# erikszasz/GaussianSplattingRegistration

Measured on AMD Instinct MI355X. Metric: Gaussians/sec through HEM level + ICP iters/sec, 2x5M-splat pair, higher is better.
Workload: dtype f32 (HEM) / f64 (ICP)

## Files before the change

gaussiansplattingregistration_amd/csrc/hem.hip:

```cpp
#include "gsr_common.h"
#include "gsr_math.h"
#include "gsr_normals.h"
#include "gsr_test_hooks.h"
#include "hem_device.h"
#include "hem_select.h"

#include <float.h>
#include <math.h>
#include <stdarg.h>
#include <stdlib.h>
#include <string.h>

#include <chrono>
#include <vector>

#include <rocprim/rocprim.hpp>

namespace gsr {

std::string& last_error() {
    static thread_local std::string s;
    return s;
}
int32_t fail(int32_t code, const char* fmt, ...) {
// ... 1774 lines not shown
        const unsigned g = gid[i];
        if ((int64_t)g >= n_global || (i > 0 && gid[i - 1] >= g)) atomicAdd(bad, 1u);
    }
}
__global__ __launch_bounds__(256) void k_gid_drop(int64_t n, const unsigned* __restrict__ bits, const int* __restrict__ wpre, unsigned* __restrict__ gid) {
    for (int64_t i = (int64_t)blockIdx.x * blockDim.x + threadIdx.x; i < n; i += (int64_t)gridDim.x * blockDim.x) {
        const unsigned g = gid[i];
        gid[i] = g - ((unsigned)wpre[g >> 5] + (unsigned)__popc(bits[g >> 5] & ((1u << (g & 31)) - 1u)));
    }
}
__global__ __launch_bounds__(256) void k_compact_u32(int64_t n, const int* __restrict__ keep, const int* __restrict__ pos, const unsigned* __restrict__ src,
                                                     unsigned* __restrict__ dst) {
    for (int64_t i = (int64_t)blockIdx.x * blockDim.x + threadIdx.x; i < n; i += (int64_t)gridDim.x * blockDim.x)
        if (keep[i]) dst[pos[i]] = src[i];
}
__global__ __launch_bounds__(256) void k_not_flag(int64_t n, const int* __restrict__ in, int* __restrict__ out) {
    for (int64_t i = (int64_t)blockIdx.x * blockDim.x + threadIdx.x; i < n; i += (int64_t)gridDim.x * blockDim.x) out[i] = in[i] ? 0 : 1;
}
__global__ void k_last_total(const int* __restrict__ pos_last, const int* __restrict__ flag_last, long long* __restrict__ out) { *out = (long long)*pos_last + *flag_last; }
__global__ void k_flip3(unsigned* __restrict__ w) { if (threadIdx.x < 3) w[threadIdx.x] = ~w[threadIdx.x]; }

__global__ __launch_bounds__(256) void k_valid(int64_t n, const float* __restrict__ xyz, const float* __restrict__ cov6,
                                               int* __restrict__ keep, const long long* __restrict__ n_dev, int* __restrict__ dropped,
                                               int* __restrict__ holes ) {
    if (n_dev) n = *n_dev;
    for (int64_t i = (int64_t)blockIdx.x * blockDim.x + threadIdx.x; i < n; i += (int64_t)gridDim.x * blockDim.x) {
        const float x = xyz[3 * i], y = xyz[3 * i + 1], z = xyz[3 * i + 2];
        s6 c = {cov6[6 * i], cov6[6 * i + 1], cov6[6 * i + 2], cov6[6 * i + 3], cov6[6 * i + 4], cov6[6 * i + 5]};
        const float d = det6(c);
        const bool bad = (x != x) || (y != y) || (z != z) || (d != d) || (d <= 0.0f);
        keep[i] = bad ? 0 : 1;
        if (bad && dropped) {
            const int slot = atomicAdd(dropped, 1);
            if (holes && slot < ERASE_MAX) holes[slot] = (int)i;
        }
    }
}

struct EraseArgs {
    float* arr[6];
    int w[6];
    uint8_t* flags;
    float* halo;
    int W;
    int tile;
    int max_tiles;
    const int* holes;
    const int* dropped;
// ... 288 lines not shown
    bool mstep_small = true;
    bool use_ell = true;
    int shard_rank = 0, shard_world = 1;
    gsr_allreduce_dev_fn shard_allreduce = nullptr;
    gsr_allgather_dev_fn shard_allgather = nullptr;
    void* shard_user = nullptr;
    DevBuf shard_send, shard_recv;
    bool sparse_path = false;
    DevBuf hitem, hfirst, part_cnt, Ac, cellStartC, cellStartI;
    DevBuf pcnt, poff, pair_child, pair_wl, spair_child, spair_wl, cstart, sumLw, oflag, pflag_in, oflag_in, prank_in, orank_in;
    DevBuf keep, kpos, scratch, draws, counters, rocprim_tmp, rocprim_tmp2, sh_tail, holes, erase_halo;
    int64_t stats[8] = {0, 0, 0, 0, 0, 0, 0, 0};
    int64_t stats_ex[8] = {0, 0, 0, 0, 0, 0, 0, 0};
    float phase_ms[8] = {0, 0, 0, 0, 0, 0, 0, 0};
    hipEvent_t ev[8] = {nullptr, nullptr, nullptr, nullptr, nullptr, nullptr, nullptr, nullptr};
    hipEvent_t evk[4] = {nullptr, nullptr, nullptr, nullptr};
    hipEvent_t evm[6] = {nullptr, nullptr, nullptr, nullptr, nullptr, nullptr};
    float kernel_ms[8] = {0, 0, 0, 0, 0, 0, 0, 0};
    struct Prologue { bool valid = false; GridParams gp; int P = 0, n_irr = 0, cblock = 0; int64_t n = 0; float ms = 0.0f; } pro;
    hipEvent_t ev_pro[2] = {nullptr, nullptr};
    int cblock = 0;
    DevBuf lvl;
    bool async_ok = true;
    bool last_level = false;
    hipStream_t side = nullptr;
    hipEvent_t ev_side = nullptr, ev_side_fork = nullptr;
    int round_trips = 0;
    int was_async = 0;
    float cell_target = 16.0f;
    int max_cells = 1 << 24;
};

namespace {

void rng_polymul(const unsigned* a, const unsigned* b, unsigned* out) {
    unsigned prod[61];
    for (int d = 0; d < 61; ++d) prod[d] = 0;
    for (int i = 0; i < 31; ++i) for (int j = 0; j < 31; ++j) prod[i + j] += a[i] * b[j];
    for (int d = 60; d >= 31; --d) { const unsigned c = prod[d]; prod[d - 3] += c; prod[d - 31] += c; }
    for (int d = 0; d < 31; ++d) out[d] = prod[d];
}
const unsigned* rng_xpow_table() {
    struct Table {
        unsigned tab[48 * 31];
        Table() {
            for (int j = 0; j < 31; ++j) tab[j] = j == 1 ? 1u : 0u;
// ... 93 lines not shown
    const unsigned long long seq = ++c->rb_seq;
    hipLaunchKernelGGL(k_collect, dim3(1), dim3(8), 0, c->stream, q, c->host_rb, seq);
    GSR_HIP(hipGetLastError());
    GSR_TRY(wait_round_trip(c, seq));
    for (int i = 0; i < q.n; ++i) out[i] = __atomic_load_n(c->host_rb + i, __ATOMIC_RELAXED);
    return GSR_OK;
}
int32_t read_back_level(gsr_hem_ctx* c, const LevelCollect& q, unsigned long long* out) {
    const unsigned long long seq = ++c->rb_seq;
    hipLaunchKernelGGL(k_level_collect, dim3(1), dim3(64), 0, c->stream, q, c->host_rb, seq);
    GSR_HIP(hipGetLastError());
    GSR_TRY(wait_round_trip(c, seq));
    for (int i = 0; i < LC_WORDS; ++i) out[i] = __atomic_load_n(c->host_rb + 16 + i, __ATOMIC_RELAXED);
    return GSR_OK;
}

#ifndef GSR_SCAN_BIG_N
#define GSR_SCAN_BIG_N (1 << 20)
#endif
using scan_cfg_big = rocprim::scan_config<256, 64, rocprim::block_load_method::block_load_transpose, rocprim::block_store_method::block_store_transpose,
                                          rocprim::block_scan_algorithm::using_warp_scan>;
using scan_cfg64_big = rocprim::scan_config<256, 32, rocprim::block_load_method::block_load_transpose, rocprim::block_store_method::block_store_transpose,
                                            rocprim::block_scan_algorithm::using_warp_scan>;
template <typename T>
int32_t exclusive_scan(gsr_hem_ctx* c, const T* in, T* out, int64_t n, bool side = false) {
    size_t bytes = 0;
    const hipStream_t s = side ? c->aux : c->stream;
    DevBuf& tmp = side ? c->rocprim_tmp2 : c->rocprim_tmp;
    if (n >= GSR_SCAN_BIG_N) {
        GSR_HIP(rocprim::exclusive_scan<scan_cfg_big>(nullptr, bytes, in, out, (T)0, (size_t)n, rocprim::plus<T>(), s));
        GSR_TRY(tmp.reserve(bytes));
        GSR_HIP(rocprim::exclusive_scan<scan_cfg_big>(tmp.p, bytes, in, out, (T)0, (size_t)n, rocprim::plus<T>(), s));
        return GSR_OK;
    }
    GSR_HIP(rocprim::exclusive_scan(nullptr, bytes, in, out, (T)0, (size_t)n, rocprim::plus<T>(), s));
    GSR_TRY(tmp.reserve(bytes));
    GSR_HIP(rocprim::exclusive_scan(tmp.p, bytes, in, out, (T)0, (size_t)n, rocprim::plus<T>(), s));
    return GSR_OK;
}

#ifndef GSR_SORT_RADIX_BITS
#define GSR_SORT_RADIX_BITS 10
#endif
#ifndef GSR_SORT_MERGE_LIMIT
#define GSR_SORT_MERGE_LIMIT (256 * 1024)
#endif
#ifndef GSR_SORT_BS
#define GSR_SORT_BS 1024
#endif
#ifndef GSR_SORT_IPT
// ... 135 lines not shown
        if (e == hipSuccess) e = hipEventCreateWithFlags(&c->ev_mjoin, hipEventDisableTiming);
        for (int i = 0; i < 4 && e == hipSuccess; ++i) e = hipEventCreate(&c->evp[i]);
        for (int i = 0; i < 2 && e == hipSuccess; ++i) e = hipEventCreate(&c->ev_pro[i]);
        if (e != hipSuccess) { delete c; return fail(GSR_E_HIP, "second stream: %s", hipGetErrorString(e)); }
    }
    {
        hipError_t e = hipHostMalloc((void**)&c->host_rb, 512, hipHostMallocMapped | hipHostMallocCoherent);
        if (e != hipSuccess) { c->host_rb = nullptr; delete c; return fail(GSR_E_HIP, "hipHostMalloc: %s", hipGetErrorString(e)); }
        memset(c->host_rb, 0, 512);
    }
    if (const char* s = getenv("GSR_HEM_ELL")) c->use_ell = atoi(s) != 0;
    if (const char* s = getenv("GSR_HEM_SUMLW")) c->sum_bucket = strcmp(s, "sort") != 0;
    if (const char* s = getenv("GSR_HEM_SPLIT")) c->split_heavy = atoi(s) != 0;
    if (const char* s = getenv("GSR_HEM_MSTEP_SMALL")) c->mstep_small = atoi(s) != 0;
    if (const char* s = getenv("GSR_HEM_MSTEP_SPLIT")) c->mstep_split = atoi(s) != 0;
    if (const char* s = getenv("GSR_HEM_SH_DIRECT")) c->sh_policy = atoi(s) != 0 ? 1 : 0;
    if (const char* s = getenv("GSR_HEM_SH_DIRECT_PAIRS")) c->sh_direct_pairs = (float)atof(s);
    if (const char* s = getenv("GSR_HEM_ROWLIST")) c->use_rowlist = atoi(s) != 0;
    if (const char* s = getenv("GSR_HEM_ROWLIST_MAX_MB")) c->rowlist_max = (size_t)(atof(s) * 1048576.0);
    if (const char* s = getenv("GSR_HEM_TIMING")) { const int v = atoi(s); c->timing = v < 0 ? 0 : (v > 2 ? 2 : v); }
    if (const char* s = getenv("GSR_HEM_SELECT_NP")) { const int v = atoi(s); c->select_np = v < 1 ? 1 : (v > SEL_NP ? SEL_NP : v); }
    if (const char* s = getenv("GSR_HEM_RB_POLL")) c->rb_poll = atoi(s) != 0;
    if (const char* s = getenv("GSR_HEM_ASYNC")) c->async_ok = atoi(s) != 0;
    if (const char* s = getenv("GSR_HEM_PARTITION_STAGE")) { const int v = atoi(s); if (v == 8192 || v == 6144 || v == 4096) c->partition_stage = v; }
    if (const char* s = getenv("GSR_HEM_PARTITION")) { c->partition_fixed = strcmp(s, "exact") != 0; c->partition_staged = strcmp(s, "walk") != 0; }
    if (const char* s = getenv("GSR_HEM_PARTITION_FACTOR")) c->partition_factor = atof(s);
    if (const char* s = getenv("GSR_HEM_CELL_TARGET")) { float v = (float)atof(s); if (v > 0.25f && v < 4096.0f) c->cell_target = v; }
    (void)hipFuncSetAttribute((const void*)k_bucket_sum, hipFuncAttributeMaxDynamicSharedMemorySize, 12 << 13);
    (void)hipFuncSetAttribute((const void*)k_bucket_hist, hipFuncAttributeMaxDynamicSharedMemorySize, SUM_MAX_BUCKETS * 4);
    (void)hipFuncSetAttribute((const void*)k_bucket_scatter, hipFuncAttributeMaxDynamicSharedMemorySize, SUM_MAX_BUCKETS * 4);
    (void)hipFuncSetAttribute((const void*)k_partition<0>, hipFuncAttributeMaxDynamicSharedMemorySize, SUM_MAX_BUCKETS * 4);
    (void)hipFuncSetAttribute((const void*)k_partition<8192>, hipFuncAttributeMaxDynamicSharedMemorySize, 1536 * 8 + 8192 * 8);
    (void)hipFuncSetAttribute((const void*)k_partition<6144>, hipFuncAttributeMaxDynamicSharedMemorySize, 3584 * 8 + 6144 * 8);
    (void)hipFuncSetAttribute((const void*)k_partition<4096>, hipFuncAttributeMaxDynamicSharedMemorySize, 5632 * 8 + 4096 * 8);
    (void)hipFuncSetAttribute((const void*)k_part_max, hipFuncAttributeMaxDynamicSharedMemorySize, 4 << 13);
    (void)hipFuncSetAttribute((const void*)k_part_acc, hipFuncAttributeMaxDynamicSharedMemorySize, 12 << 13);
    (void)hipFuncSetAttribute((const void*)k_erase_shift, hipFuncAttributeMaxDynamicSharedMemorySize, 12288 * 4);
    *out = c;
    return GSR_OK;
}

int32_t gsr_hem_destroy(gsr_hem_ctx* c) {
    if (!c) return GSR_OK;
    (void)hipSetDevice(c->device);
    unborrow_level0(c);
    for (DevBuf& b : c->spare) b.release();
// ... 478 lines not shown
            }
            GSR_TRY(gsr_comm_allreduce(c->comm, c->gbits.p, words, GSR_DT_U32, GSR_OP_SUM, (void*)st));
            hipLaunchKernelGGL(k_bits_popc, dim3(stride_grid(words)), blk, 0, st, words, c->gbits.as<unsigned>(), c->wcnt.as<int>());
            GSR_TRY(exclusive_scan<int>(c, c->wcnt.as<int>(), c->wpre.as<int>(), words));
            if (dropped > 0) {
                GSR_TRY(c->grank.reserve((size_t)n_pre * 4));
                hipLaunchKernelGGL(k_compact_u32, dim3(stride_grid(n_pre)), blk, 0, st, n_pre, c->keep.as<int>(), c->kpos.as<int>(), c->gid_next.as<unsigned>(), c->grank.as<unsigned>());
                c->gid_next.swap(c->grank);
            }
            if (O.n > 0) hipLaunchKernelGGL(k_gid_drop, dim3(stride_grid(O.n)), blk, 0, st, O.n, c->gbits.as<unsigned>(), c->wpre.as<int>(), c->gid_next.as<unsigned>());
            n_glob_next = n_pre_glob - dg;
        }
        c->part_stats[6] = dg;
        return GSR_OK;
    }
};

}

namespace {

constexpr int32_t GSR_RETRY_SYNC = -1000;

struct LevelRun {
    gsr_hem_ctx* c;
    hipStream_t st;
    Level& L;
    Level& O;
    const bool dbg_sync, part, sharded;
    bool spec = false;
    const int sh_policy;
    const int64_t n_own;
    int64_t n;
    const int F, RSH;
    PartLevel pl;
    const dim3 blk{256};
    dim3 grd;
    GridParams gp;
    int P_all = 0, P = 0, n_irr = 0;
    int* cnt = nullptr;
    long long* lvl = nullptr;
    const float4* rec_src = nullptr;
    bool ranks_forked = false, sh_pending = false, sh_launched = false, flags_forked = false;
    SelectArgs sa;
    size_t Pm = 1;
    int own_lo = 0, own_hi = 0;
    int64_t M = 0;
    unsigned long long cand = 0, cap_pairs = 0;
    const int64_t* seg = nullptr;
    const unsigned* pc = nullptr;
    const float* pw = nullptr;
    int bshift = 0, nbuckets = 0;
    int* overflow_flag = nullptr;
    bool fixed_tried = false;
    int64_t n_orph = 0, n_pre = 0, out_cap = 0;
    bool out_active = false;
    uint64_t rng_pos0 = 0;
    int64_t dropped = 0, P_glob = 0, O_glob = 0, n_pre_glob = 0, n_glob_next = 0;
    float pro_ms = 0.0f;

    LevelRun(gsr_hem_ctx* ctx, bool allow_async)
        : c(ctx), st(ctx->stream), L(ctx->cur), O(ctx->nxt), dbg_sync(getenv("GSR_HEM_DEBUG_SYNC") != nullptr), part(ctx->comm != nullptr),
          sharded(ctx->shard_world > 1 && ctx->shard_allreduce != nullptr), sh_policy(ctx->comm == nullptr ? ctx->sh_policy : 0), n_own(ctx->cur.n), n(ctx->cur.n), F(ctx->cur.F), RSH((ctx->cur.F + 3) & ~3) {
        spec = allow_async;
        pl.c = c; pl.st = st; pl.n_own = n_own;
        memset(&sa, 0, sizeof(sa));
    }
    ~LevelRun() {
        if (out_active) for (int i = 0; i < 5; ++i) { DevBuf* b = level_big(c->nxt, i); b->p = nullptr; b->cap = 0; b->swap(c->spare_out[i]); }
    }

    int32_t run(int64_t* n_out, int64_t* n_dropped);
    int32_t grid_phase();
    int32_t select_phase();
    int32_t sums_phase();
    int32_t sums_fixed();
    int32_t sums_exact();
    int32_t compact_pairs();
    int32_t output_ranks();
    int32_t open_output();
    int32_t mstep_phase();
    int32_t flags_and_validity();
    int32_t compact_erased(int64_t n_keep);
    int32_t erase_in_place(int64_t rows_bound, bool may_allocate, int64_t alloc_rows = 0);
    bool erase_on_device = false;
    int32_t launch_gather_sh(bool fork);
    int32_t widen_scan(const unsigned* cnt_in, int64_t* off, int64_t count);
    int32_t total_of(const int64_t* off, const unsigned* cnt_in, int64_t count, int64_t* out);
};

struct WidenU32 { __device__ __host__ int64_t operator()(unsigned v) const { return (int64_t)v; } };
int32_t LevelRun::widen_scan(const unsigned* cnt_in, int64_t* off, int64_t count) {
    auto in = rocprim::make_transform_iterator(cnt_in, WidenU32());
    size_t bytes = 0;
    if (count >= GSR_SCAN_BIG_N) {
        GSR_HIP(rocprim::exclusive_scan<scan_cfg64_big>(nullptr, bytes, in, off, (int64_t)0, (size_t)count, rocprim::plus<int64_t>(), st));
        GSR_TRY(c->rocprim_tmp.reserve(bytes));
        GSR_HIP(rocprim::exclusive_scan<scan_cfg64_big>(c->rocprim_tmp.p, bytes, in, off, (int64_t)0, (size_t)count, rocprim::plus<int64_t>(), st));
        return GSR_OK;
    }
    GSR_HIP(rocprim::exclusive_scan(nullptr, bytes, in, off, (int64_t)0, (size_t)count, rocprim::plus<int64_t>(), st));
    GSR_TRY(c->rocprim_tmp.reserve(bytes));
    GSR_HIP(rocprim::exclusive_scan(c->rocprim_tmp.p, bytes, in, off, (int64_t)0, (size_t)count, rocprim::plus<int64_t>(), st));
    return GSR_OK;
}
int32_t LevelRun::total_of(const int64_t* off, const unsigned* cnt_in, int64_t count, int64_t* out) {
    Collect q;
    q.n = 2;
    q.src[0] = off + (count - 1); q.bytes[0] = 8;
    q.src[1] = cnt_in + (count - 1); q.bytes[1] = 4;
    unsigned long long w[8];
    GSR_TRY(read_back(c, q, w));
    *out = (int64_t)w[0] + (int64_t)(unsigned)w[1];
    return GSR_OK;
}
// ... 41 lines not shown
            hipLaunchKernelGGL(k_flip3, dim3(1), dim3(64), 0, st, c->bbox.as<unsigned>());
            GSR_TRY(gsr_comm_allreduce(c->comm, c->bbox.p, 6, GSR_DT_U32, GSR_OP_MAX, (void*)st));
            hipLaunchKernelGGL(k_flip3, dim3(1), dim3(64), 0, st, c->bbox.as<unsigned>());
        }
        hipLaunchKernelGGL(k_hist, dim3(stride_grid(n) > 512 ? 512 : stride_grid(n)), blk, 0, st, n, L.xyz.as<float>(), c->bbox.as<unsigned>(), c->hist.as<unsigned>(),
                           (const long long*)nullptr);
        if (part) GSR_TRY(gsr_comm_allreduce(c->comm, c->hist.p, 3 * HIST_BINS, GSR_DT_U32, GSR_OP_SUM, (void*)st));
        hipLaunchKernelGGL(k_grid_params, dim3(1), dim3(64), 0, st, c->bbox.as<unsigned>(), c->hist.as<unsigned>(), part ? c->n_global : n, c->cell_target,
                           c->max_cells, c->gparams.as<GridParams>(), (const long long*)nullptr);
        static_assert(sizeof(GridParams) == 40, "GridParams is read back as five 8-byte words");
        Collect q;
        q.n = 7;
        for (int i = 0; i < 5; ++i) { q.src[i] = (const char*)c->gparams.p + 8 * i; q.bytes[i] = 8; }
        q.src[5] = c->bbox.as<unsigned>() + 6; q.src[6] = c->bbox.as<unsigned>() + 7;
        q.bytes[5] = q.bytes[6] = 4;
        unsigned long long w[8];
        GSR_TRY(read_back(c, q, w));
        memcpy(&gp, w, sizeof(gp));
        P_all = (int)(unsigned)w[5]; n_irr = (int)(unsigned)w[6];
    }
    overflow_flag = cnt + 12;
    c->stats[5] = gp.ncells;
    GSR_TRY(c->pflag_in.reserve(n * 4)); GSR_TRY(c->oflag_in.reserve(n * 4)); GSR_TRY(c->prank_in.reserve(n * 4)); GSR_TRY(c->orank_in.reserve(n * 4));
    if (!part && c->aux && c->ev_pre) {
        GSR_HIP(hipEventRecord(c->ev_fork, st)); GSR_HIP(hipStreamWaitEvent(c->aux, c->ev_fork, 0));
        hipLaunchKernelGGL(k_flags_in, grd, blk, 0, c->aux, n, n_own, L.is_parent.as<uint8_t>(), c->pflag_in.as<int>(), c->oflag_in.as<int>());
        GSR_TRY(exclusive_scan<int>(c, c->pflag_in.as<int>(), c->prank_in.as<int>(), n, true));
        GSR_HIP(hipEventRecord(c->ev_pre, c->aux));
        ranks_forked = true;
    }

    rec_src = c->rec.as<float4>();
    if (part) {
        GSR_TRY(pl.halo(gp, L, F, n));
        grd = dim3(stride_grid(n));
        rec_src = c->rec_loc.as<float4>();
    }
    GSR_TRY(c->keys.reserve(n * 4)); GSR_TRY(c->idx.reserve(n * 4)); GSR_TRY(c->skeys.reserve(n * 4)); GSR_TRY(c->order.reserve(n * 4));
    if (part) {
        GSR_TRY(c->perm.reserve(n * 4));
        hipLaunchKernelGGL(k_iota, grd, blk, 0, st, n, c->idx.as<unsigned>());
        GSR_TRY(sort_pairs<unsigned>(c, c->gid_loc.as<unsigned>(), c->skeys.as<unsigned>(), c->idx.as<unsigned>(), c->perm.as<unsigned>(), n, bits_for(c->n_global + 1)));
        hipLaunchKernelGGL(k_keys_rec, grd, blk, 0, st, n, rec_src, c->perm.as<unsigned>(), c->gparams.as<GridParams>(), c->keys.as<unsigned>(), c->idx.as<unsigned>());
    } else
        hipLaunchKernelGGL(k_keys, grd, blk, 0, st, n, L.xyz.as<float>(), c->gparams.as<GridParams>(), c->keys.as<unsigned>(), c->idx.as<unsigned>());
    GSR_TRY(sort_pairs<unsigned>(c, c->keys.as<unsigned>(), c->skeys.as<unsigned>(), c->idx.as<unsigned>(), c->order.as<unsigned>(), n,
                                 bits_for(gp.ncells)));
// ... 144 lines not shown
        if (sparse) {
            if (!spec) {
                const size_t Cm = (size_t)(cand > 0 ? cand : 1);
                GSR_TRY(c->sp_child.reserve(Cm * 4)); GSR_TRY(c->sp_wl.reserve(Cm * 4));
                cap_pairs = (unsigned long long)(std::min(c->sp_child.cap, c->sp_wl.cap) / 4);
            }
            sa.cap_pairs = cap_pairs;
            sa.poff = c->coff.as<int64_t>(); sa.pair_child = c->sp_child.as<unsigned>(); sa.pair_wl = c->sp_wl.as<float>();
            GSR_TIME1(c->evk[2], st);
            GSR_CHECKPOINT("spans + ordering");
            GSR_LAUNCH_SELECT(SEL_SPARSE);
            GSR_CHECKPOINT("k_select<SPARSE>");
            GSR_TIME1(c->evk[3], st);
        } else {
            GSR_TIME1(c->evk[0], st);
            GSR_LAUNCH_SELECT(SEL_COUNT);
            GSR_TIME1(c->evk[1], st);
        }
        GSR_TRY(widen_scan(c->pcnt.as<unsigned>(), c->poff.as<int64_t>(), P));
        if (!spec) GSR_TRY(total_of(c->poff.as<int64_t>(), c->pcnt.as<unsigned>(), P, &M));
        if ((spec || M > 0) && sparse && sa.heavy_blocks)
            hipLaunchKernelGGL(k_join_parts, dim3(1024), blk, 0, st, sa.nheavy, sa.porder, c->coff.as<int64_t>(), sa.hfirst, sa.part_cnt,
                               c->pcap.as<unsigned>(), sa.part_p, c->sp_child.as<unsigned>(), c->sp_wl.as<float>());
        if (!sh_launched) { GSR_TRY(launch_gather_sh(c->aux2 != nullptr)); sh_launched = true; }
        if (spec || M > 0) {
            if (!sparse) {
                const size_t Mm = (size_t)(M > 0 ? M : 1);
                GSR_TRY(c->pair_child.reserve(Mm * 4)); GSR_TRY(c->pair_wl.reserve(Mm * 4));
                sa.poff = c->poff.as<int64_t>(); sa.pair_child = c->pair_child.as<unsigned>(); sa.pair_wl = c->pair_wl.as<float>();
                if (sa.heavy_blocks)
                    hipLaunchKernelGGL(k_fill_const<int>, dim3(1), dim3(1), 0, st, (int64_t)1, sa.hq + 1, (int)(SEL_HEAVY_BLOCKS * WPB));
                GSR_TIME1(c->evk[2], st);
                GSR_LAUNCH_SELECT(SEL_FILL);
                GSR_TIME1(c->evk[3], st);
            }
        }
        c->sparse_path = sparse;
        c->stats_ex[1] = sparse ? 1 : 0;
    } else if (spec) {
        return GSR_RETRY_SYNC;
    }
#undef GSR_LAUNCH_SELECT
    c->stats[1] = M;
    GSR_CHECKPOINT("selection");
    GSR_TIME(c->ev[2], st);
    return GSR_OK;
}
// ... 158 lines not shown
        if (need > 0) {
            for (int i = 0; i < 5; ++i) {
                DevBuf* b = level_big(O, i);
                b->swap(c->spare_out[i]);
                b->p = c->out_ptr[i] ? c->out_ptr[i] : c->out_ptr[0]; b->cap = (size_t)-1;
            }
            out_active = true;
        }
    }
    GSR_TRY(O.reserve(need, F));
    out_cap = out_active ? std::min<int64_t>(c->out_rows, n + (int64_t)P) : need;
    if (spec) out_cap = std::min(out_cap, need);
    O.n = spec ? 0 : n_pre; O.F = F;
    if (spec)
        hipLaunchKernelGGL(k_level_tail, dim3(1), dim3(1), 0, st, n, P, c->orank_in.as<int>(), c->oflag_in.as<int>(), (long long)out_cap, lvl, cnt + 2);
    return GSR_OK;
}

int32_t LevelRun::mstep_phase() {
    const long long* n_pre_dev = spec ? lvl : nullptr;
    const int* sh_mode = reinterpret_cast<const int*>(lvl + 3);
    rng_pos0 = c->rng_pos;
    const int64_t n_draw = spec ? out_cap : n_pre;
    if (!part && c->aux && n_draw > 0) {
        GSR_HIP(hipEventRecord(c->ev_fork, st)); GSR_HIP(hipStreamWaitEvent(c->aux, c->ev_fork, 0));
        GSR_TRY(O.is_parent.reserve((size_t)n_draw));
        GSR_TRY(draw_flags_raw(c, n_draw, O.is_parent.as<uint8_t>(), c->aux, n_pre_dev));
        GSR_HIP(hipEventRecord(c->ev_join, c->aux));
        flags_forked = true;
    }
    if (!sh_launched) { GSR_TRY(launch_gather_sh(false)); sh_launched = true; }
    if (sh_pending) { GSR_HIP(hipStreamWaitEvent(st, c->ev_sh_join, 0)); sh_pending = false; }
    if (P > 0) {
        MstepArgs ma;
        memset(&ma, 0, sizeof(ma));
        ma.geo = c->geo.as<float4>(); ma.RSH = RSH;
        ma.sh_mode_p = sh_mode; ma.sh_own = L.sh.as<float>(); ma.sh_sorted = c->shs.as<float>();
        ma.sh_last = part ? 0xffffffffu : (unsigned)(n - 1); ma.sh_tail = c->sh_tail.as<float>();
        ma.pair_child = pc; ma.pair_wl = pw;
        ma.P = P; ma.F = F;
        ma.small = c->mstep_small ? 1 : 0;
        const unsigned* mporder = (spec || M > 0) ? c->porder.as<unsigned>() : nullptr;
        ma.xcd = mporder ? 1 : 0;
        ma.nheavy = mporder ? cnt + 8 : nullptr;
        GSR_TRY(c->mhdr.reserve(Pm * sizeof(MstepHeader)));
        const bool msplit = spec || M > MSTEP_SEG;
        if (msplit) {
// ... 3 lines not shown
            GSR_TRY(c->mh_scratch.reserve(cap_items * (size_t)(16 + RSH) * 4));
        }
        unsigned* hcount = (unsigned*)cnt;
        hipLaunchKernelGGL(k_mstep_headers, dim3(stride_grid(P)), blk, 0, st, P, mporder, c->plist.as<unsigned>(), seg,
                           c->pcnt.as<unsigned>(), c->order.as<unsigned>(), c->prank_in.as<int>(), c->A.as<float4>(), own_lo, own_hi,
                           c->mhdr.as<MstepHeader>(), (unsigned*)cnt + 15, (unsigned)MSTEP_SEG, msplit ? hcount : (unsigned*)nullptr,
                           c->mh_list.as<uint4>(), c->mh_items.as<uint2>());
        ma.hdr = c->mhdr.as<MstepHeader>();
        ma.split = c->mstep_split ? 1 : 0;
        ma.hcount = hcount; ma.hlist = c->mh_list.as<uint4>(); ma.hitems = c->mh_items.as<uint2>(); ma.hscratch = c->mh_scratch.as<float>();
        ma.o_xyz = O.xyz.as<float>(); ma.o_color = O.color.as<float>(); ma.o_cov6 = O.cov6.as<float>();
        ma.o_opacity = O.opacity.as<float>(); ma.o_weight = O.weight.as<float>(); ma.o_sh = O.sh.as<float>();
        const int nq = RSH >> 2;
        hipStream_t hst = st;
        if (msplit && c->aux) {
            GSR_HIP(hipEventRecord(c->ev_mfork, st)); GSR_HIP(hipStreamWaitEvent(c->aux, c->ev_mfork, 0));
            hst = c->aux;
        }
#define GSR_LAUNCH_MSTEP(G)                                                                                              \
    {                                                                                                                    \
        if (msplit && hst != st) {                                                                                       \
            hipLaunchKernelGGL((k_mstep<G, 1, true>), dim3(2048), dim3(64), 0, hst, ma);                                 \
            hipLaunchKernelGGL(k_mstep_heavy_finish, dim3(256), dim3(64), 0, hst, ma);                                   \
            GSR_HIP(hipEventRecord(c->ev_mjoin, hst));                                                                   \
        }                                                                                                                \
        hipLaunchKernelGGL((k_mstep<G, 1>), dim3(8 * ceil_div(ceil_div(P, MSTEP_K), 8)), dim3(64), 0, st, ma);           \
        if (msplit && hst == st) {                                                                                       \
            hipLaunchKernelGGL((k_mstep<G, 1, true>), dim3(2048), dim3(64), 0, st, ma);                                  \
            hipLaunchKernelGGL(k_mstep_heavy_finish, dim3(256), dim3(64), 0, st, ma);                                    \
        }                                                                                                                \
    }
        GSR_TIME1(c->evm[0], st);
        if (nq == 0) { GSR_LAUNCH_MSTEP(0) }
        else if (nq <= 1 * MSTEP_NV) { GSR_LAUNCH_MSTEP(1) }
        else if (nq <= 2 * MSTEP_NV) { GSR_LAUNCH_MSTEP(2) }
        else if (nq <= 4 * MSTEP_NV) { GSR_LAUNCH_MSTEP(4) }
        else if (nq <= 8 * MSTEP_NV) { GSR_LAUNCH_MSTEP(8) }
        else if (nq <= 16 * MSTEP_NV) { GSR_LAUNCH_MSTEP(16) }
        else { GSR_LAUNCH_MSTEP(32) }
#undef GSR_LAUNCH_MSTEP
        if (msplit && hst != st) GSR_HIP(hipStreamWaitEvent(st, c->ev_mjoin, 0));
        GSR_TIME1(c->evm[1], st);
    }
    hipLaunchKernelGGL(k_orphan_rows, dim3(stride_grid(n_own)), blk, 0, st, n_own, P, c->oflag_in.as<int>(), c->orank_in.as<int>(), L.xyz.as<float>(), L.color.as<float>(),
                       L.cov6.as<float>(), L.opacity.as<float>(), L.weight.as<float>(), L.sh.as<float>(), F, O.xyz.as<float>(), O.color.as<float>(),
                       O.cov6.as<float>(), O.opacity.as<float>(), O.weight.as<float>(), O.sh.as<float>(), (int64_t)(spec ? out_cap : n_pre));
// ... 8 lines not shown
                               c->order.as<unsigned>(), c->prank_in.as<int>(), c->shard_send.as<float>(), O.xyz.as<float>(), O.color.as<float>(),
                               O.cov6.as<float>(), O.opacity.as<float>(), O.weight.as<float>(), O.sh.as<float>());
        GSR_HIP(hipStreamSynchronize(st));
        if (c->shard_allgather(c->shard_send.p, c->shard_recv.p, (int64_t)chunk_bytes, c->shard_user) != 0)
            return fail(GSR_E_INVALID, "gsr_hem_run_level: all-gather callback failed (merged components)");
        for (int r = 0; r < W; ++r) {
            if (r == c->shard_rank) continue;
            const int lo = (int)((int64_t)P * r / W), hi = (int)((int64_t)P * (r + 1) / W);
            if (hi > lo)
                hipLaunchKernelGGL((k_shard_rows<false>), dim3(stride_grid((int64_t)(hi - lo) * RW)), blk, 0, st, lo, hi - lo, F, c->plist.as<unsigned>(),
                                   c->order.as<unsigned>(), c->prank_in.as<int>(), c->shard_recv.as<float>() + (size_t)r * chunk * RW, O.xyz.as<float>(),
                                   O.color.as<float>(), O.cov6.as<float>(), O.opacity.as<float>(), O.weight.as<float>(), O.sh.as<float>());
        }
    }
    P_glob = P; O_glob = n_orph;
    if (part) GSR_TRY(pl.global_ranks(P, n_pre, P_glob, O_glob));
    n_pre_glob = P_glob + O_glob;
    GSR_CHECKPOINT("M-step + orphans");
    GSR_TIME(c->ev[4], st);
    return GSR_OK;
}

int32_t LevelRun::erase_in_place(int64_t rows_bound, bool may_allocate, int64_t alloc_rows) {
    const int tile0 = std::min(256, 12288 / std::max(F, 6));
    const auto halo_bytes = [&](int64_t rows) { return (size_t)((rows + tile0 - 1) / tile0 + 1) * ERASE_MAX * ((size_t)(14 + F) * 4 + 1) + 64; };
    {
        const size_t need = halo_bytes(rows_bound);
        if (!may_allocate && c->erase_halo.cap < need) {
            hipLaunchKernelGGL(k_fill_const<long long>, dim3(1), dim3(1), 0, st, (int64_t)1, lvl + 4, (long long)0);
            return GSR_OK;
        }
    }
    erase_on_device = true;
    EraseArgs ea;
    memset(&ea, 0, sizeof(ea));
    float* arrs[6] = {O.xyz.as<float>(), O.color.as<float>(), O.cov6.as<float>(), O.opacity.as<float>(), O.weight.as<float>(), O.sh.as<float>()};
    const int ws[6] = {3, 3, 6, 1, 1, F};
    for (int q = 0; q < 6; ++q) { ea.arr[q] = arrs[q]; ea.w[q] = ws[q]; }
    ea.flags = O.is_parent.as<uint8_t>();
    ea.W = 14 + F;
    ea.tile = std::min(256, 12288 / std::max(F, 6));
    ea.max_tiles = (int)((rows_bound + ea.tile - 1) / ea.tile) + 1;
    GSR_TRY(c->erase_halo.reserve(halo_bytes(std::max(rows_bound, alloc_rows))));
    ea.halo = c->erase_halo.as<float>();
    ea.holes = c->holes.as<int>(); ea.dropped = cnt + 3; ea.n_pre_p = lvl; ea.n_keep_out = lvl + 4;
    const int g = std::min(ea.max_tiles, 2048);
    hipLaunchKernelGGL(k_erase_save, dim3(g), blk, 0, st, ea);
    hipLaunchKernelGGL(k_erase_shift, dim3(g), blk, (size_t)12288 * 4, st, ea);
    GSR_HIP(hipGetLastError());
    return GSR_OK;
}

int32_t LevelRun::compact_erased(int64_t n_keep) {
    Level& T = c->tmp;
    const dim3 g2(stride_grid(n_pre));
    GSR_TRY(T.reserve(n_keep, F));
    T.n = n_keep; T.F = F;
    const int* keep = c->keep.as<int>();
    const int* pos = c->kpos.as<int>();
    hipLaunchKernelGGL(k_compact_rows, dim3(stride_grid(n_pre * 3)), blk, 0, st, n_pre, 3, keep, pos, O.xyz.as<float>(), T.xyz.as<float>());
    hipLaunchKernelGGL(k_compact_rows, dim3(stride_grid(n_pre * 3)), blk, 0, st, n_pre, 3, keep, pos, O.color.as<float>(), T.color.as<float>());
    hipLaunchKernelGGL(k_compact_rows, dim3(stride_grid(n_pre * 6)), blk, 0, st, n_pre, 6, keep, pos, O.cov6.as<float>(), T.cov6.as<float>());
    hipLaunchKernelGGL(k_compact_rows, g2, blk, 0, st, n_pre, 1, keep, pos, O.opacity.as<float>(), T.opacity.as<float>());
    hipLaunchKernelGGL(k_compact_rows, g2, blk, 0, st, n_pre, 1, keep, pos, O.weight.as<float>(), T.weight.as<float>());
    if (F > 0)
        hipLaunchKernelGGL(k_compact_rows4, dim3(stride_grid(n_pre * ((F + 3) / 4))), blk, 0, st, n_pre, F, keep, pos, O.sh.as<float>(), T.sh.as<float>());
    hipLaunchKernelGGL(k_compact_bytes, g2, blk, 0, st, n_pre, keep, pos, O.is_parent.as<uint8_t>(), T.is_parent.as<uint8_t>());
    if (out_active) {
        const size_t row_bytes[5] = {12, 12, 24, 4, (size_t)F * 4};
        for (int i = 0; i < 5; ++i)
            if (row_bytes[i] > 0 && n_keep > 0)
                GSR_HIP(hipMemcpyAsync(level_big(O, i)->p, level_big(T, i)->p, (size_t)n_keep * row_bytes[i], hipMemcpyDeviceToDevice, st));
        O.weight.swap(T.weight); O.is_parent.swap(T.is_parent);
        O.n = n_keep;
    } else
        O.swap(T);
    return GSR_OK;
}

int32_t LevelRun::flags_and_validity() {
    if (part) {
        GSR_TRY(c->allflags.reserve((size_t)(n_pre_glob > 0 ? n_pre_glob : 1)));
        GSR_TRY(draw_flags_raw(c, n_pre_glob, c->allflags.as<uint8_t>()));
        if (n_pre > 0)
            hipLaunchKernelGGL(k_gather_bytes, dim3(stride_grid(n_pre)), blk, 0, st, n_pre, c->gid_next.as<unsigned>(), c->allflags.as<uint8_t>(), O.is_parent.as<uint8_t>());
    } else if (flags_forked) {
        GSR_HIP(hipStreamWaitEvent(st, c->ev_join, 0));
    } else {
        GSR_TRY(draw_flags(c, O));
    }
    dropped = 0;
    if (n_pre > 0) {
        GSR_TRY(c->keep.reserve(n_pre * 4)); GSR_TRY(c->kpos.reserve(n_pre * 4));
        const dim3 g2(stride_grid(n_pre));
        GSR_TRY(c->holes.reserve(ERASE_MAX * 4));
        hipLaunchKernelGGL(k_valid, g2, blk, 0, st, n_pre, O.xyz.as<float>(), O.cov6.as<float>(), c->keep.as<int>(), (const long long*)nullptr, cnt + 3, c->holes.as<int>());
        if (part) GSR_TRY(exclusive_scan<int>(c, c->keep.as<int>(), c->kpos.as<int>(), n_pre));
        {
            Collect q;
            q.n = 2;
            q.src[0] = cnt + 3; q.src[1] = cnt + 15;
            q.bytes[0] = q.bytes[1] = 4;
            unsigned long long w[8];
            GSR_TRY(read_back(c, q, w));
            dropped = (int64_t)(unsigned)w[0];
            if (P > 0) c->stats_ex[5] = (int64_t)(unsigned)w[1];
        }
        if (dropped > 0 && dropped <= ERASE_MAX && !part) {
            hipLaunchKernelGGL(k_fill_const<long long>, dim3(1), dim3(1), 0, st, (int64_t)1, lvl, (long long)n_pre);
            GSR_TRY(erase_in_place(n_pre, true, n));
            O.n = n_pre - dropped;
        } else if (dropped > 0) {
            if (!part) GSR_TRY(exclusive_scan<int>(c, c->keep.as<int>(), c->kpos.as<int>(), n_pre));
            GSR_TRY(compact_erased(n_pre - dropped));
        }
    }
    n_glob_next = n_pre_glob;
    if (part) GSR_TRY(pl.drop_erased(O, n_pre, n_pre_glob, dropped, n_glob_next));
    GSR_CHECKPOINT("flags + validity");
    return GSR_OK;
}

int32_t LevelRun::run(int64_t* n_out, int64_t* n_dropped) {
    memset(c->stats, 0, sizeof(c->stats));
    memset(c->stats_ex, 0, sizeof(c->stats_ex));
    memset(c->part_stats, 0, sizeof(c->part_stats));
    c->stats[6] = n;
    if (part) {
        pl.W = gsr_comm_world(c->comm); pl.me = gsr_comm_rank(c->comm);
        const unsigned code = c->shard_world > 1 ? 4u : (pl.W > 8 ? 3u : (n >= (1ll << 30) ? 2u : 0u));
        GSR_TRY(pl.agree_on_preconditions(n, code));
    }
    if (n >= (1ll << 30)) return fail(GSR_E_INVALID, "gsr_hem_run_level: %lld components (the candidate records carry the sorted position in 30 bits)", (long long)n);
    if (n == 0) {
        if (n_out) *n_out = 0;
        if (n_dropped) *n_dropped = 0;
        return GSR_OK;
    }
    spec = spec && !part && !sharded && !dbg_sync && c->sum_bucket && c->partition_fixed && !c->partition_overflowed && c->partition_factor == 0.0 &&
           c->split_heavy && getenv("GSR_HEM_SPARSE_GB") == nullptr && c->aux != nullptr &&
           std::min(c->sp_child.cap, c->sp_wl.cap) >= (size_t)4096 && std::min(c->spair_child.cap / sizeof(slot_t), c->spair_wl.cap / 4) >= (size_t)4096;
    grd = dim3(stride_grid(n));
    GSR_TIME1(c->ev[0], st);
    GSR_TRY(grid_phase());
    GSR_TRY(select_phase());
    GSR_TRY(sums_phase());
    GSR_TRY(output_ranks());
    GSR_TRY(open_output());
    GSR_TRY(mstep_phase());

    unsigned long long w[LC_WORDS];
    bool have_next = false;
    const bool want_pro = !c->last_level;
    const int cb_next = c->cblock ^ 1;
    LevelCollect q;
    memset(&q, 0, sizeof(q));
    q.cnt = cnt; q.gp = c->gparams.as<GridParams>(); q.bbox = c->bbox.as<unsigned>();
    if (P > 0) { q.coff = c->coff.as<int64_t>(); q.pcap = c->pcap.as<unsigned>(); q.poff = c->poff.as<int64_t>(); q.pcnt = c->pcnt.as<unsigned>(); q.P = P; }
    if (spec) {
        if (flags_forked) GSR_HIP(hipStreamWaitEvent(st, c->ev_join, 0));
        GSR_TRY(c->keep.reserve((size_t)out_cap * 4)); GSR_TRY(c->kpos.reserve((size_t)out_cap * 4));
        GSR_TRY(c->holes.reserve(ERASE_MAX * 4));
        hipLaunchKernelGGL(k_valid, dim3(stride_grid(out_cap)), blk, 0, st, out_cap, O.xyz.as<float>(), O.cov6.as<float>(), c->keep.as<int>(), (const long long*)lvl, cnt + 3,
                           c->holes.as<int>());
        GSR_TRY(erase_in_place(out_cap, false));
        GSR_TIME1(c->ev[5], st);
        if (want_pro) GSR_TRY(enqueue_prologue(c, O, out_cap, erase_on_device ? lvl + 4 : lvl, cb_next));
        q.lvl = lvl;
        GSR_TRY(read_back_level(c, q, w));
        if (w[LC_FLAGS] != 0ull) return GSR_RETRY_SYNC;
        cand = w[LC_CAND]; M = (int64_t)w[LC_PAIRS]; n_orph = (int64_t)w[LC_ORPHANS]; n_pre = (int64_t)w[LC_NPRE];
        c->stats[4] = (int64_t)cand; c->stats[1] = M; c->stats[2] = n_orph;
        c->stats_ex[3] = (int64_t)w[LC_HEAVY]; c->stats_ex[4] = (int64_t)w[LC_ITEMS]; c->stats_ex[5] = (int64_t)w[LC_MAXPAIRS];
        c->rng_pos = rng_pos0 + (uint64_t)n_pre;
        O.n = n_pre;
        P_glob = P; O_glob = n_orph; n_pre_glob = n_pre; n_glob_next = n_pre;
        dropped = (int64_t)w[LC_DROPPED];
        have_next = dropped == 0 || (erase_on_device && dropped <= ERASE_MAX);
        if (have_next) O.n = n_pre - dropped;
        else if (dropped <= ERASE_MAX) {
            GSR_TRY(erase_in_place(n_pre, true, out_cap));
            O.n = n_pre - dropped;
        } else {
            GSR_TRY(exclusive_scan<int>(c, c->keep.as<int>(), c->kpos.as<int>(), n_pre));
            GSR_TRY(compact_erased(n_pre - dropped));
        }
    } else {
        GSR_TRY(flags_and_validity());
// ... 251 lines not shown
```

Baseline: 578.6 million.

## Add single-block scan for small inputs and fold side-stream forks on small levels

Adds a one-block, 1024-thread warp-scan kernel that replaces the rocprim exclusive scans (including the widening u32→i64 scan) when the input fits in 64K items and is 16-byte aligned. This avoids rocprim's temp-size query and multi-kernel launches. Levels under 128K components skip the aux-stream fork for the flags scan and the gather-SH launch. The parent-flag draw is moved onto the heavy-mstep side stream so one fork/join serves both. The erase kernel launch is skipped when the halo buffer is too small, with k_valid clearing the keep count itself. The aim is to cut launch, event and stream-sync overhead on the many small coarse levels, at the cost of more code paths and some lost overlap.

```diff
diff --git a/gaussiansplattingregistration_amd/csrc/hem.hip b/gaussiansplattingregistration_amd/csrc/hem.hip
--- a/gaussiansplattingregistration_amd/csrc/hem.hip
+++ b/gaussiansplattingregistration_amd/csrc/hem.hip
@@ -1820,8 +1820,10 @@
 
 __global__ __launch_bounds__(256) void k_valid(int64_t n, const float* __restrict__ xyz, const float* __restrict__ cov6,
                                                int* __restrict__ keep, const long long* __restrict__ n_dev, int* __restrict__ dropped,
-                                               int* __restrict__ holes ) {
+                                               int* __restrict__ holes ,
+                                               long long* __restrict__ clear_p ) {
     if (n_dev) n = *n_dev;
+    if (clear_p && blockIdx.x == 0 && threadIdx.x == 0) *clear_p = 0;
     for (int64_t i = (int64_t)blockIdx.x * blockDim.x + threadIdx.x; i < n; i += (int64_t)gridDim.x * blockDim.x) {
         const float x = xyz[3 * i], y = xyz[3 * i + 1], z = xyz[3 * i + 2];
         s6 c = {cov6[6 * i], cov6[6 * i + 1], cov6[6 * i + 2], cov6[6 * i + 3], cov6[6 * i + 4], cov6[6 * i + 5]};
@@ -2156,6 +2158,7 @@
     int cblock = 0;
     DevBuf lvl;
     bool async_ok = true;
+    bool fold = true;
     bool last_level = false;
     hipStream_t side = nullptr;
     hipEvent_t ev_side = nullptr, ev_side_fork = nullptr;
@@ -2295,10 +2298,85 @@
                                           rocprim::block_scan_algorithm::using_warp_scan>;
 using scan_cfg64_big = rocprim::scan_config<256, 32, rocprim::block_load_method::block_load_transpose, rocprim::block_store_method::block_store_transpose,
                                             rocprim::block_scan_algorithm::using_warp_scan>;
+#ifndef GSR_SCAN_ONE_N
+#define GSR_SCAN_ONE_N 65536
+#endif
+constexpr int SCAN_ONE_TILES = GSR_SCAN_ONE_N / (16 * 256);
+static_assert(SCAN_ONE_TILES >= 1 && SCAN_ONE_TILES <= 16 && SCAN_ONE_TILES * 16 * 256 == GSR_SCAN_ONE_N, "GSR_SCAN_ONE_N: 16 waves x whole tiles of 256 items, at most 16 each");
+template <typename TIn, typename TOut, int TILES>
+__global__ __launch_bounds__(1024) void k_scan_one(int n, const TIn* __restrict__ in, TOut* __restrict__ out) {
+    static_assert(sizeof(TIn) == 4 && (sizeof(TOut) == 4 || sizeof(TOut) == 8), "k_scan_one: 4-byte items, 4- or 8-byte sums");
+    using WaveScan = rocprim::warp_scan<TOut, 64>;
+    __shared__ typename WaveScan::storage_type s_scan[16];
+    __shared__ TOut s_tot[16];
+    const int lane = threadIdx.x & 63, wv = threadIdx.x >> 6;
+    const int per_wave = (n + 16 * 256 - 1) / (16 * 256) * 256;
+    const int base = wv * per_wave + lane * 4;
+    uint4 v[TILES];
+#pragma unroll
+    for (int t = 0; t < TILES; ++t) {
+        const int i = base + t * 256;
+        const bool mine = t * 256 < per_wave;
+        if (mine && i + 3 < n) {
+            v[t] = *reinterpret_cast<const uint4*>(in + i);
+        } else {
+            v[t].x = mine && i < n ? (unsigned)in[i] : 0u;
+            v[t].y = mine && i + 1 < n ? (unsigned)in[i + 1] : 0u;
+            v[t].z = mine && i + 2 < n ? (unsigned)in[i + 2] : 0u;
+            v[t].w = mine && i + 3 < n ? (unsigned)in[i + 3] : 0u;
+        }
+    }
+    TOut mine_sum = 0;
+#pragma unroll
+    for (int t = 0; t < TILES; ++t) mine_sum = mine_sum + ((TOut)(TIn)v[t].x + (TOut)(TIn)v[t].y + (TOut)(TIn)v[t].z + (TOut)(TIn)v[t].w);
+    {
+        TOut inc, tot;
+        WaveScan().inclusive_scan(mine_sum, inc, tot, s_scan[wv]);
+        if (lane == 0) s_tot[wv] = tot;
+    }
+    __syncthreads();
+#pragma unroll
+    for (int t = 0; t < TILES; ++t) asm volatile("" : "+v"(v[t].x), "+v"(v[t].y), "+v"(v[t].z), "+v"(v[t].w));
+    TOut carry = 0;
+    for (int u = 0; u < wv; ++u) carry = carry + s_tot[u];
+#pragma unroll
+    for (int t = 0; t < TILES; ++t) {
+        const int i = base + t * 256;
+        if (!(t * 256 < per_wave)) break;
+        const TOut s = (TOut)(TIn)v[t].x + (TOut)(TIn)v[t].y + (TOut)(TIn)v[t].z + (TOut)(TIn)v[t].w;
+        TOut inc, tot;
+        WaveScan().inclusive_scan(lane == 0 ? s + carry : s, inc, tot, s_scan[wv]);
+        carry = tot;
+        if (i >= n) continue;
+        TOut e[4];
+        e[0] = inc - s;
+        e[1] = e[0] + (TOut)(TIn)v[t].x; e[2] = e[1] + (TOut)(TIn)v[t].y; e[3] = e[2] + (TOut)(TIn)v[t].z;
+        if (i + 3 < n) {
+            if constexpr (sizeof(TOut) == 4) {
+                *reinterpret_cast<uint4*>(out + i) = make_uint4((unsigned)e[0], (unsigned)e[1], (unsigned)e[2], (unsigned)e[3]);
+            } else {
+                *reinterpret_cast<ulonglong2*>(out + i) = make_ulonglong2((unsigned long long)e[0], (unsigned long long)e[1]);
+                *reinterpret_cast<ulonglong2*>(out + i + 2) = make_ulonglong2((unsigned long long)e[2], (unsigned long long)e[3]);
+            }
+        } else {
+#pragma unroll
+            for (int k = 0; k < 4; ++k) if (i + k < n) out[i + k] = e[k];
+        }
+    }
+}
+template <typename TIn, typename TOut>
+bool scan_one(gsr_hem_ctx* c, const TIn* in, TOut* out, int64_t n, hipStream_t s) {
+    constexpr int TILES = sizeof(TOut) == 4 ? SCAN_ONE_TILES : (SCAN_ONE_TILES + 1) / 2;
+    if (!c->fold || n <= 0 || n > (int64_t)TILES * 16 * 256 || (((uintptr_t)in | (uintptr_t)out) & 15u) != 0 || (const void*)in == (const void*)out) return false;
+    hipLaunchKernelGGL((k_scan_one<TIn, TOut, TILES>), dim3(1), dim3(1024), 0, s, (int)n, in, out);
+    return true;
+}
+
 template <typename T>
 int32_t exclusive_scan(gsr_hem_ctx* c, const T* in, T* out, int64_t n, bool side = false) {
     size_t bytes = 0;
     const hipStream_t s = side ? c->aux : c->stream;
+    if (scan_one<T, T>(c, in, out, n, s)) return GSR_OK;
     DevBuf& tmp = side ? c->rocprim_tmp2 : c->rocprim_tmp;
     if (n >= GSR_SCAN_BIG_N) {
         GSR_HIP(rocprim::exclusive_scan<scan_cfg_big>(nullptr, bytes, in, out, (T)0, (size_t)n, rocprim::plus<T>(), s));
@@ -2480,6 +2558,7 @@
     if (const char* s = getenv("GSR_HEM_SELECT_NP")) { const int v = atoi(s); c->select_np = v < 1 ? 1 : (v > SEL_NP ? SEL_NP : v); }
     if (const char* s = getenv("GSR_HEM_RB_POLL")) c->rb_poll = atoi(s) != 0;
     if (const char* s = getenv("GSR_HEM_ASYNC")) c->async_ok = atoi(s) != 0;
+    if (const char* s = getenv("GSR_HEM_FOLD")) c->fold = atoi(s) != 0;
     if (const char* s = getenv("GSR_HEM_PARTITION_STAGE")) { const int v = atoi(s); if (v == 8192 || v == 6144 || v == 4096) c->partition_stage = v; }
     if (const char* s = getenv("GSR_HEM_PARTITION")) { c->partition_fixed = strcmp(s, "exact") != 0; c->partition_staged = strcmp(s, "walk") != 0; }
     if (const char* s = getenv("GSR_HEM_PARTITION_FACTOR")) c->partition_factor = atof(s);
@@ -3004,6 +3083,9 @@
 
 constexpr int32_t GSR_RETRY_SYNC = -1000;
 
+#ifndef GSR_INLINE_N
+#define GSR_INLINE_N (128 * 1024)
+#endif
 struct LevelRun {
     gsr_hem_ctx* c;
     hipStream_t st;
@@ -3024,6 +3106,8 @@
     long long* lvl = nullptr;
     const float4* rec_src = nullptr;
     bool ranks_forked = false, sh_pending = false, sh_launched = false, flags_forked = false;
+    bool flags_joined = false;
+    bool small_level = false;
     SelectArgs sa;
     size_t Pm = 1;
     int own_lo = 0, own_hi = 0;
@@ -3065,6 +3149,10 @@
     int32_t flags_and_validity();
     int32_t compact_erased(int64_t n_keep);
     int32_t erase_in_place(int64_t rows_bound, bool may_allocate, int64_t alloc_rows = 0);
+    size_t erase_halo_bytes(int64_t rows) const {
+        const int tile0 = std::min(256, 12288 / std::max(F, 6));
+        return (size_t)((rows + tile0 - 1) / tile0 + 1) * ERASE_MAX * ((size_t)(14 + F) * 4 + 1) + 64;
+    }
     bool erase_on_device = false;
     int32_t launch_gather_sh(bool fork);
     int32_t widen_scan(const unsigned* cnt_in, int64_t* off, int64_t count);
@@ -3073,6 +3161,7 @@
 
 struct WidenU32 { __device__ __host__ int64_t operator()(unsigned v) const { return (int64_t)v; } };
 int32_t LevelRun::widen_scan(const unsigned* cnt_in, int64_t* off, int64_t count) {
+    if (scan_one<unsigned, int64_t>(c, cnt_in, off, count, st)) return GSR_OK;
     auto in = rocprim::make_transform_iterator(cnt_in, WidenU32());
     size_t bytes = 0;
     if (count >= GSR_SCAN_BIG_N) {
@@ -3160,7 +3249,7 @@
     overflow_flag = cnt + 12;
     c->stats[5] = gp.ncells;
     GSR_TRY(c->pflag_in.reserve(n * 4)); GSR_TRY(c->oflag_in.reserve(n * 4)); GSR_TRY(c->prank_in.reserve(n * 4)); GSR_TRY(c->orank_in.reserve(n * 4));
-    if (!part && c->aux && c->ev_pre) {
+    if (!part && c->aux && c->ev_pre && !small_level) {
         GSR_HIP(hipEventRecord(c->ev_fork, st)); GSR_HIP(hipStreamWaitEvent(c->aux, c->ev_fork, 0));
         hipLaunchKernelGGL(k_flags_in, grd, blk, 0, c->aux, n, n_own, L.is_parent.as<uint8_t>(), c->pflag_in.as<int>(), c->oflag_in.as<int>());
         GSR_TRY(exclusive_scan<int>(c, c->pflag_in.as<int>(), c->prank_in.as<int>(), n, true));
@@ -3351,7 +3440,7 @@
         if ((spec || M > 0) && sparse && sa.heavy_blocks)
             hipLaunchKernelGGL(k_join_parts, dim3(1024), blk, 0, st, sa.nheavy, sa.porder, c->coff.as<int64_t>(), sa.hfirst, sa.part_cnt,
                                c->pcap.as<unsigned>(), sa.part_p, c->sp_child.as<unsigned>(), c->sp_wl.as<float>());
-        if (!sh_launched) { GSR_TRY(launch_gather_sh(c->aux2 != nullptr)); sh_launched = true; }
+        if (!sh_launched) { GSR_TRY(launch_gather_sh(c->aux2 != nullptr && !small_level)); sh_launched = true; }
         if (spec || M > 0) {
             if (!sparse) {
                 const size_t Mm = (size_t)(M > 0 ? M : 1);
@@ -3556,7 +3645,9 @@
     const int* sh_mode = reinterpret_cast<const int*>(lvl + 3);
     rng_pos0 = c->rng_pos;
     const int64_t n_draw = spec ? out_cap : n_pre;
-    if (!part && c->aux && n_draw > 0) {
+    const bool flags_side = !part && c->aux && n_draw > 0;
+    const bool one_fork = c->fold && flags_side && P > 0 && (spec || M > MSTEP_SEG);
+    if (flags_side && !one_fork) {
         GSR_HIP(hipEventRecord(c->ev_fork, st)); GSR_HIP(hipStreamWaitEvent(c->aux, c->ev_fork, 0));
         GSR_TRY(O.is_parent.reserve((size_t)n_draw));
         GSR_TRY(draw_flags_raw(c, n_draw, O.is_parent.as<uint8_t>(), c->aux, n_pre_dev));
@@ -3606,6 +3697,11 @@
         if (msplit && hst != st) {                                                                                       \
             hipLaunchKernelGGL((k_mstep<G, 1, true>), dim3(2048), dim3(64), 0, hst, ma);                                 \
             hipLaunchKernelGGL(k_mstep_heavy_finish, dim3(256), dim3(64), 0, hst, ma);                                   \
+            if (one_fork) {                                                                                              \
+                GSR_TRY(O.is_parent.reserve((size_t)n_draw));                                                            \
+                GSR_TRY(draw_flags_raw(c, n_draw, O.is_parent.as<uint8_t>(), hst, n_pre_dev));                           \
+                flags_forked = flags_joined = true;                                                                      \
+            }                                                                                                            \
             GSR_HIP(hipEventRecord(c->ev_mjoin, hst));                                                                   \
         }                                                                                                                \
         hipLaunchKernelGGL((k_mstep<G, 1>), dim3(8 * ceil_div(ceil_div(P, MSTEP_K), 8)), dim3(64), 0, st, ma);           \
@@ -3660,10 +3756,8 @@
 }
 
 int32_t LevelRun::erase_in_place(int64_t rows_bound, bool may_allocate, int64_t alloc_rows) {
-    const int tile0 = std::min(256, 12288 / std::max(F, 6));
-    const auto halo_bytes = [&](int64_t rows) { return (size_t)((rows + tile0 - 1) / tile0 + 1) * ERASE_MAX * ((size_t)(14 + F) * 4 + 1) + 64; };
     {
-        const size_t need = halo_bytes(rows_bound);
+        const size_t need = erase_halo_bytes(rows_bound);
         if (!may_allocate && c->erase_halo.cap < need) {
             hipLaunchKernelGGL(k_fill_const<long long>, dim3(1), dim3(1), 0, st, (int64_t)1, lvl + 4, (long long)0);
             return GSR_OK;
@@ -3679,7 +3773,7 @@
     ea.W = 14 + F;
     ea.tile = std::min(256, 12288 / std::max(F, 6));
     ea.max_tiles = (int)((rows_bound + ea.tile - 1) / ea.tile) + 1;
-    GSR_TRY(c->erase_halo.reserve(halo_bytes(std::max(rows_bound, alloc_rows))));
+    GSR_TRY(c->erase_halo.reserve(erase_halo_bytes(std::max(rows_bound, alloc_rows))));
     ea.halo = c->erase_halo.as<float>();
     ea.holes = c->holes.as<int>(); ea.dropped = cnt + 3; ea.n_pre_p = lvl; ea.n_keep_out = lvl + 4;
     const int g = std::min(ea.max_tiles, 2048);
@@ -3723,7 +3817,7 @@
         if (n_pre > 0)
             hipLaunchKernelGGL(k_gather_bytes, dim3(stride_grid(n_pre)), blk, 0, st, n_pre, c->gid_next.as<unsigned>(), c->allflags.as<uint8_t>(), O.is_parent.as<uint8_t>());
     } else if (flags_forked) {
-        GSR_HIP(hipStreamWaitEvent(st, c->ev_join, 0));
+        if (!flags_joined) GSR_HIP(hipStreamWaitEvent(st, c->ev_join, 0));
     } else {
         GSR_TRY(draw_flags(c, O));
     }
@@ -3732,7 +3826,7 @@
         GSR_TRY(c->keep.reserve(n_pre * 4)); GSR_TRY(c->kpos.reserve(n_pre * 4));
         const dim3 g2(stride_grid(n_pre));
         GSR_TRY(c->holes.reserve(ERASE_MAX * 4));
-        hipLaunchKernelGGL(k_valid, g2, blk, 0, st, n_pre, O.xyz.as<float>(), O.cov6.as<float>(), c->keep.as<int>(), (const long long*)nullptr, cnt + 3, c->holes.as<int>());
+        hipLaunchKernelGGL(k_valid, g2, blk, 0, st, n_pre, O.xyz.as<float>(), O.cov6.as<float>(), c->keep.as<int>(), (const long long*)nullptr, cnt + 3, c->holes.as<int>(), (long long*)nullptr);
         if (part) GSR_TRY(exclusive_scan<int>(c, c->keep.as<int>(), c->kpos.as<int>(), n_pre));
         {
             Collect q;
@@ -3779,6 +3873,7 @@
            c->split_heavy && getenv("GSR_HEM_SPARSE_GB") == nullptr && c->aux != nullptr &&
            std::min(c->sp_child.cap, c->sp_wl.cap) >= (size_t)4096 && std::min(c->spair_child.cap / sizeof(slot_t), c->spair_wl.cap / 4) >= (size_t)4096;
     grd = dim3(stride_grid(n));
+    small_level = c->fold && n < (int64_t)GSR_INLINE_N;
     GSR_TIME1(c->ev[0], st);
     GSR_TRY(grid_phase());
     GSR_TRY(select_phase());
@@ -3796,12 +3891,13 @@
     q.cnt = cnt; q.gp = c->gparams.as<GridParams>(); q.bbox = c->bbox.as<unsigned>();
     if (P > 0) { q.coff = c->coff.as<int64_t>(); q.pcap = c->pcap.as<unsigned>(); q.poff = c->poff.as<int64_t>(); q.pcnt = c->pcnt.as<unsigned>(); q.P = P; }
     if (spec) {
-        if (flags_forked) GSR_HIP(hipStreamWaitEvent(st, c->ev_join, 0));
+        if (flags_forked && !flags_joined) GSR_HIP(hipStreamWaitEvent(st, c->ev_join, 0));
         GSR_TRY(c->keep.reserve((size_t)out_cap * 4)); GSR_TRY(c->kpos.reserve((size_t)out_cap * 4));
         GSR_TRY(c->holes.reserve(ERASE_MAX * 4));
+        const bool count_only = c->fold && c->erase_halo.cap < erase_halo_bytes(out_cap);
         hipLaunchKernelGGL(k_valid, dim3(stride_grid(out_cap)), blk, 0, st, out_cap, O.xyz.as<float>(), O.cov6.as<float>(), c->keep.as<int>(), (const long long*)lvl, cnt + 3,
-                           c->holes.as<int>());
-        GSR_TRY(erase_in_place(out_cap, false));
+                           c->holes.as<int>(), count_only ? lvl + 4 : (long long*)nullptr);
+        if (!count_only) GSR_TRY(erase_in_place(out_cap, false));
         GSR_TIME1(c->ev[5], st);
         if (want_pro) GSR_TRY(enqueue_prologue(c, O, out_cap, erase_on_device ? lvl + 4 : lvl, cb_next));
         q.lvl = lvl;
```

Result: no change. 579.9 million (median of 3 runs) (+0.2%).
